# noveens/reviews4rec

Measured on AMD Instinct MI355X. Metric: train ratings/sec, higher is better.
Workload: dtype f32

## Files before the change

### include/r4r.h

```cpp
#ifndef R4R_H
#define R4R_H

#include <stddef.h>
#include <stdint.h>

#ifdef __cplusplus
extern "C" {
#endif

#define R4R_OK 0
#define R4R_ERR_ARG (-1)
#define R4R_ERR_LAUNCH (-2)
#define R4R_ERR_WORKSPACE (-3)

int r4r_version(void);
const char *r4r_last_error(void);

size_t r4r_textcnn_ws_bytes(int64_t N, int T, int E, int F, int64_t V);
int r4r_textcnn_fwd(const float *table, int64_t V, const int64_t *idx,
                    const float *conv_w, const float *conv_b,
                    float *pooled, int32_t *argmax,
                    void *ws, size_t ws_bytes,
                    int64_t N, int T, int E, int F, void *stream);

// ... 27 lines not shown
int r4r_add(const float *a, const float *b, float *out, int64_t n, void *stream);

int r4r_fm_fwd(const float *x, const float *V, const float *lin_w, const float *lin_b,
               float *out, int64_t N, int n, int k, void *stream);
int r4r_fm_bwd(const float *x, const float *V, const float *lin_w, const float *g_out,
               float *g_x, float *g_V, float *g_lin_w, float *g_lin_b,
               int64_t N, int n, int k, void *stream);

int r4r_embed_gather(const float *table, const int64_t *idx, float *out,
                     int64_t R, int D, int64_t n, void *stream);
int r4r_embed_scatter_add(const float *g_out, const int64_t *idx, float *g_table,
                          int64_t R, int D, int64_t n, void *stream);
int r4r_embed_scatter_add_ordered(const float *g_out, const int64_t *idx, float *g_table,
                                  int64_t R, int D, int64_t n, void *stream);

int r4r_rowdot_fwd(const float *a, const float *c, float *out, int64_t N, int D, void *stream);
int r4r_rowdot_bwd(const float *a, const float *c, const float *g_out, float *g_a, float *g_c,
                   int64_t N, int D, void *stream);
int r4r_bias_head_fwd(const float *r, const float *user_bias, const float *item_bias,
                      const float *global_bias, const int64_t *uid, const int64_t *iid,
                      float *out, int64_t N, void *stream);
int r4r_bias_head_bwd(const float *g_out, const int64_t *uid, const int64_t *iid,
                      float *g_user_bias, float *g_item_bias, float *g_global,
                      int64_t RU, int64_t RI, int64_t N, void *stream);

size_t r4r_narre_attn_ws_bytes(int64_t N, int R, int L);
int r4r_narre_attn_fwd(const float *x, const float *other, const float *W0, const float *b0,
                       const float *w3, const float *b3, const float *mult,
                       float *out, float *h_save, float *a_save,
                       int64_t N, int R, int L, void *stream);
int r4r_narre_attn_bwd(const float *x, const float *other, const float *W0, const float *w3,
                       const float *mult, const float *h_save, const float *a_save,
                       const float *g_out,
                       float *g_x, float *g_other, float *g_W0, float *g_b0, float *g_w3, float *g_b3,
                       void *ws, size_t ws_bytes,
                       int64_t N, int R, int L, void *stream);

int r4r_mse_fwd_bwd(const float *out, const float *y, float *se, float *g_out,
                    int64_t N, float denom, void *stream);

int r4r_sqdist_mean_fwd(const float *a, const float *b, float *out, int64_t N, int L, void *stream);
int r4r_sqdist_mean_bwd(const float *a, const float *b, const float *g_out, float *g_a, float *g_b,
                        int64_t N, int L, void *stream);

int r4r_adam_chunk_elems(void);
int r4r_adam_multi(int ntensor, const uint64_t *p, const uint64_t *g, const uint64_t *m, const uint64_t *v,
                   const int64_t *numel, float lr, double beta1, double beta2, float eps,
                   float weight_decay, int64_t step, const int64_t *step_dev, void *stream);
int r4r_adam_gathered(float *p, const float *gathered, int world, float *g_sum, float *m, float *v,
                      int64_t numel, float lr, double beta1, double beta2, float eps,
                      float weight_decay, int64_t step, void *stream);
int r4r_adam_gathered_guarded(float *p, const float *gathered, int world, float *g_sum, float *m, float *v,
                              int64_t numel, float lr, double beta1, double beta2, float eps,
                              float weight_decay, int64_t step, const uint32_t *abort_word, void *stream);

int r4r_peer_segment_create(int64_t bytes, void **ptr, uint8_t *handle);
int r4r_peer_segment_open(const uint8_t *handle, void **ptr);
int r4r_peer_segment_close(void *ptr);
int r4r_peer_segment_destroy(void *ptr);
int r4r_peer_push(const float *src, int64_t numel, const uint64_t *peer_dst, const uint64_t *peer_flags,
                  uint32_t *arrive, int rank, int world, uint32_t epoch, const uint32_t *wait_flags,
                  uint32_t *timed_out, double timeout_s, void *stream);
int r4r_peer_wait(const uint32_t *flags, int world, uint32_t epoch, uint32_t *timed_out, double timeout_s, void *stream);


#define R4R_CONV_AUTO 0
#define R4R_CONV_DIRECT 1
#define R4R_CONV_PROJECT 2
int r4r_deepconn_nparam(void);
int r4r_deepconn_layout(int E, int L, int64_t *offsets, int64_t *sizes, int64_t *total);
size_t r4r_deepconn_ws_bytes(int64_t B, int T, int E, int L, int64_t V);
size_t r4r_deepconn_ws_mult_offset(int64_t B, int T, int E, int L, int64_t V);
size_t r4r_deepconn_ws_count_offset(int64_t B, int T, int E, int L, int64_t V, int tower, int buffer);
int r4r_deepconn_step(const float *table, int64_t V, const int64_t *user_idx, const int64_t *item_idx,
                      const float *y, float *flat_p, float *flat_g,
                      float *pred, float *se, float *sse_accum,
                      void *ws, size_t ws_bytes,
                      int64_t B, int T, int E, int L,
                      float dropout_p, int training, uint64_t seed, uint64_t offset,
                      float inv_denom, int conv_algo, int token_buffer, int tokens_ready,
                      const int64_t *next_user_idx, const int64_t *next_item_idx,
                      float *flat_m, float *flat_v, float lr, double beta1, double beta2, float eps,
                      float weight_decay, int64_t adam_step, void *stream);
int r4r_deepconn_tokens(const int64_t *user_idx, const int64_t *item_idx, void *ws, size_t ws_bytes,
                        int64_t B, int T, int E, int L, int64_t V, int conv_algo, int token_buffer,
                        int discard, void *stream);

#define R4R_TIMING_TEXTCNN_FWD 0
#define R4R_TIMING_TEXTCNN_WGRAD 1
#define R4R_TIMING_ADAM 2
#define R4R_TIMING_PROJ_GEMM 3
#define R4R_TIMING_PROJ_GATHER 4
#define R4R_TIMING_SLOTS 8
int r4r_timing_enable(int slot_mask);
int r4r_timing_read(int slot, double *total_ms, int64_t *count, int reset);

size_t r4r_mf_ws_bytes(int64_t B, int D, int64_t n_users, int64_t n_items);
size_t r4r_mf_ws_persist_bytes(int64_t B, int D, int64_t n_users, int64_t n_items);
size_t r4r_mf_ws_mult_offset(int64_t B, int D, int64_t n_users, int64_t n_items);
size_t r4r_mf_ws_grad_offset(int64_t B, int D, int64_t n_users, int64_t n_items, int which);
int r4r_mf_step(const int64_t *uid, const int64_t *iid, const float *y,
                const uint64_t *p, const uint64_t *m, const uint64_t *v,
                int64_t n_users, int64_t n_items, int D,
                float *pred, float *se, float *sse_accum, void *ws, size_t ws_bytes, int64_t B,
                float dropout_p, int training, uint64_t seed, uint64_t offset, float inv_denom,
                int sweep_period, int64_t sweep_base, int sweep_all,
                float lr, double beta1, double beta2, float eps, float weight_decay, int64_t adam_step,
                void *stream);

int r4r_mf_rows_flush(const uint64_t *p, const uint64_t *m, const uint64_t *v,
                      int64_t n_users, int64_t n_items, int D, void *ws, size_t ws_bytes, int64_t B,
                      int sweep_period, int64_t sweep_base,
                      float lr, double beta1, double beta2, float eps, float weight_decay, int64_t adam_step,
                      void *stream);
size_t r4r_mf_ws_flag_offset(int64_t B, int D, int64_t n_users, int64_t n_items);

int r4r_sse_accumulate(const float *se, int64_t n, float *accum, void *stream);

size_t r4r_mf_dp_block_bytes(int64_t B_pad, int D);
int r4r_mf_grad(const int64_t *uid, const int64_t *iid, const float *y, const uint64_t *p,
                const uint64_t *m, const uint64_t *v,
                int64_t n_users, int64_t n_items, int D, float *pred, float *se, void *block, float *mult,
                int64_t B, int64_t B_pad, float dropout_p, int training, uint64_t seed, uint64_t offset,
                float inv_denom, void *ws, int sweep_period, int64_t sweep_base,
                float lr, double beta1, double beta2, float eps, float weight_decay, int64_t adam_step,
                void *stream);
int r4r_mf_apply(const void *blocks, int world, int64_t B_pad, const uint64_t *p, const uint64_t *m,
                 const uint64_t *v, int64_t n_users, int64_t n_items, int D, void *ws, size_t ws_bytes,
                 int sweep_period, int64_t sweep_base, int sweep_all,
                 const float *se, int64_t se_n, float *sse_accum,
                 float lr, double beta1, double beta2, float eps, float weight_decay, int64_t adam_step,
                 void *stream);
int r4r_mf_grad_push(const int64_t *uid, const int64_t *iid, const float *y, const uint64_t *p,
                     const uint64_t *m, const uint64_t *v,
                     int64_t n_users, int64_t n_items, int D, float *pred, float *se, float *mult,
                     int64_t B, int64_t B_pad, float dropout_p, int training, uint64_t seed, uint64_t offset,
                     float inv_denom, void *ws, int sweep_period, int64_t sweep_base,
                     float lr, double beta1, double beta2, float eps, float weight_decay, int64_t adam_step,
                     const uint64_t *peer_dst, const uint64_t *peer_flags, uint32_t *arrive, int rank, int world,
                     uint32_t epoch, void *stream);
int r4r_mf_apply_peer(const void *blocks, int world, int64_t B_pad, const uint64_t *p, const uint64_t *m,
                      const uint64_t *v, int64_t n_users, int64_t n_items, int D, void *ws, size_t ws_bytes,
                      int sweep_period, int64_t sweep_base, int sweep_all,
                      const float *se, int64_t se_n, float *sse_accum,
                      float lr, double beta1, double beta2, float eps, float weight_decay, int64_t adam_step,
                      const uint32_t *wait_flags, uint32_t epoch, uint32_t *timed_out, double timeout_s,
                      void *stream);

size_t r4r_dp_block_bytes(int nfields, const int *widths, int64_t B_pad);
int r4r_dp_pack(int nfields, const uint64_t *src, const int *widths, const int *pad_ones, int64_t n,
                int64_t B_pad, void *block, void *stream);
int r4r_dp_unpack(int nfields, const uint64_t *dst, const int *widths, const void *blocks, int world,
                  int64_t B_pad, void *stream);

int r4r_narre_nparam(void);
int r4r_narre_layout(int E, int L, int64_t *offsets, int64_t *sizes, int64_t *total);
size_t r4r_narre_ws_bytes(int64_t B, int R, int T, int E, int L, int64_t V, int64_t n_users, int64_t n_items);
size_t r4r_narre_ws_offset(int64_t B, int R, int T, int E, int L, int64_t V, int64_t n_users, int64_t n_items,
                           int which);
int r4r_narre_step(const float *table, int64_t V,
                   const int64_t *user_reviews, const int64_t *item_reviews,
                   const int64_t *reviewed_items, const int64_t *users_who_reviewed,
                   const int64_t *uid, const int64_t *iid, const float *y,
                   float *flat_p, float *flat_g, float *flat_m, float *flat_v,
                   const uint64_t *rows_p, const uint64_t *rows_m, const uint64_t *rows_v,
                   int64_t n_users, int64_t n_items,
// ... 295 lines not shown
```

### reviews4rec_amd/csrc/engine.hip

```cpp
#include <stdlib.h>

#include "trace_device.h"
#include "textcnn.h"
#include "wgrad_device.h"
#include "tokens_device.h"
#include "adam_device.h"

namespace r4r {

constexpr int F_CONV = 100;
constexpr int FM_K = 8;
constexpr int MAX_L = 128;

enum { P_UCW = 0, P_UCB, P_UFW, P_UFB, P_ICW, P_ICB, P_IFW, P_IFB, P_FMV, P_FMLW, P_FMLB, P_GB, P_COUNT };

struct Layout {
    int64_t off[P_COUNT], size[P_COUNT], total;
};

static Layout make_layout(int E, int L) {
    Layout lay;
    const int64_t sz[P_COUNT] = {(int64_t)F_CONV * 3 * E, F_CONV, (int64_t)L * F_CONV, L,
                                 (int64_t)F_CONV * 3 * E, F_CONV, (int64_t)L * F_CONV, L,
                                 (int64_t)2 * L * FM_K, 2 * L, 1, 1};
    int64_t o = 0;
    for (int i = 0; i < P_COUNT; ++i) {
        lay.off[i] = o;
        lay.size[i] = sz[i];
        o += (sz[i] + 31) & ~(int64_t)31;
    }
    lay.total = o;
    return lay;
}

struct HeadArgs {
    const float *pmax[2]; const int *parg[2];
    const float *fc_w[2]; const float *fc_b[2];
    const float *V, *lin_w, *lin_b, *gbias;
    const float *y;
    float *pooled[2]; int *argmax[2];
    float *g_pooled[2];
    float *mult;
    float *x, *s, *g, *gz;
    float *pred, *se;
    int64_t B;
    int L, tiles, training, want_grad;
    float p_drop, inv_denom;
    uint64_t seed, offset;
};


constexpr int HEAD_MAX_TILES = 8;

#define SEL2(arr, s) ((s) ? (arr)[1] : (arr)[0])
HEAD_TRACE_DEFINE(r4r_debug_dc_head_trace)
template <int ML>
__global__ __launch_bounds__(256) void deepconn_head_wg_kernel(HeadArgs a) {
    HEAD_STAMP(0)
    constexpr int N2 = 2 * ML, PARTS = 256 / N2;
    __shared__ float sw[2][ML][F_CONV + 1];
    __shared__ float sfb[N2], slw[N2], sz[N2];
    __shared__ float sV[N2][FM_K];
    __shared__ float sp[2][F_CONV + 4];
    __shared__ float red[N2][PARTS + 1];
    const int tid = threadIdx.x, lane = tid & 63, w = tid >> 6;
    const int64_t b = blockIdx.x;
    const int L = a.L, n = 2 * L;
    const float lin_b0 = a.lin_b[0], gbias0 = a.gbias[0], yb = a.y ? a.y[b] : 0.f;

    constexpr int FQ = F_CONV / 4;
    typedef float hq4 __attribute__((ext_vector_type(4)));
    constexpr int WREGS = (2 * ML * FQ + 255) / 256;
    hq4 wreg[WREGS];
    const int wtot = 2 * L * FQ;
#pragma unroll
    for (int k = 0; k < WREGS; ++k) {
        const int i = min(tid + 256 * k, wtot - 1);
        const int t = i >= L * FQ;
        wreg[k] = *reinterpret_cast<const hq4 *>(SEL2(a.fc_w, t) + 4 * (i - t * L * FQ));
    }
    const int tn = min(tid, n - 1);
    const float fbreg = SEL2(a.fc_b, tn >= L)[tn - (tn >= L ? L : 0)];
    const float lwreg = a.lin_w[tn];
    constexpr int VREGS = (N2 * FM_K + 255) / 256;
    float vreg[VREGS];
#pragma unroll
    for (int k = 0; k < VREGS; ++k) vreg[k] = a.V[min(tid + 256 * k, n * FM_K - 1)];

    {
        const int t = w >> 1, f = lane + 64 * (w & 1), fc = min(f, F_CONV - 1);
        float best = -INFINITY;
        int bp = -1;
        if (a.tiles <= HEAD_MAX_TILES) {
            float v[HEAD_MAX_TILES];
            int pp[HEAD_MAX_TILES];
#pragma unroll
            for (int k = 0; k < HEAD_MAX_TILES; ++k) {
                const size_t o = ((size_t)b * a.tiles + min(k, a.tiles - 1)) * NP + fc;
                v[k] = SEL2(a.pmax, t)[o];
                pp[k] = SEL2(a.parg, t)[o];
            }
#pragma unroll
            for (int k = 0; k < HEAD_MAX_TILES; ++k)
                if (v[k] > best) { best = v[k]; bp = pp[k]; }
        } else {
            for (int k0 = 0; k0 < a.tiles; k0 += HEAD_MAX_TILES) {
                float v[HEAD_MAX_TILES];
                int pp[HEAD_MAX_TILES];
#pragma unroll
                for (int k = 0; k < HEAD_MAX_TILES; ++k) {
                    const bool in = k0 + k < a.tiles;
                    const size_t o = ((size_t)b * a.tiles + (in ? k0 + k : 0)) * NP + fc;
                    v[k] = in ? SEL2(a.pmax, t)[o] : -INFINITY;
                    pp[k] = SEL2(a.parg, t)[o];
                }
#pragma unroll
                for (int k = 0; k < HEAD_MAX_TILES; ++k)
                    if (v[k] > best) { best = v[k]; bp = pp[k]; }
            }
        }
        if (!(best > 0.f)) { best = 0.f; bp = -1; }
        if (f < F_CONV) {
            sp[t][f] = best;
            SEL2(a.pooled, t)[b * F_CONV + f] = best;
            SEL2(a.argmax, t)[b * F_CONV + f] = bp;
        }
    }
    HEAD_STAMP(1)
#pragma unroll
    for (int k = 0; k < WREGS; ++k) {
        const int i = tid + 256 * k;
        if (i < wtot) {
            const int t = i >= L * FQ, r = i - t * L * FQ, l = r / FQ, f0 = 4 * (r - l * FQ);
#pragma unroll
            for (int c = 0; c < 4; ++c) sw[t][l][f0 + c] = wreg[k][c];
        }
    }
    if (tid < n) { sfb[tid] = fbreg; slw[tid] = lwreg; }
#pragma unroll
    for (int k = 0; k < VREGS; ++k) {
// ... 31 lines not shown
            if (a.training && a.p_drop > 0.f && i < n) {
                const uint32_t r = philox_first_word(a.offset + (uint64_t)(b * n + i), a.seed);
                const float uu = (float)(r >> 8) * (1.0f / 16777216.0f);
                mult[u] = (uu >= a.p_drop) ? 1.f / (1.f - a.p_drop) : 0.f;
            }
            xi[u] *= mult[u];
        }
        float inter = 0.f;
        float sk_keep[FM_K];
#pragma unroll
        for (int k = 0; k < FM_K; ++k) {
            float pv = 0.f, pv2 = 0.f, vv[NI];
#pragma unroll
            for (int u = 0; u < NI; ++u) {
                const int i = lane + 64 * u;
                vv[u] = (i < n) ? sV[i][k] : 0.f;
                pv += xi[u] * vv[u];
                pv2 += xi[u] * xi[u] * vv[u] * vv[u];
            }
            const float sk = wave_sum(pv);
            const float s2 = wave_sum(pv2);
            inter += sk * sk - s2;
#pragma unroll
            for (int u = 0; u < NI; ++u) gacc[u] += sk * vv[u] - xi[u] * vv[u] * vv[u];
            sk_keep[k] = sk;
        }
        float pl = 0.f;
#pragma unroll
        for (int u = 0; u < NI; ++u) pl += xi[u] * lw[u];
        const float lin = wave_sum(pl);
        const float pred = (0.5f * inter + lin + lin_b0) + gbias0;
        if (lane == 0) a.pred[b] = pred;
        if (has_y) {
            const float d = pred - yb;
            if (lane == 0) a.se[b] = d * d;
            if (want) {
                const float g = 2.f * d * a.inv_denom;
#pragma unroll
                for (int u = 0; u < NI; ++u) {
                    const int i = lane + 64 * u;
                    const float gx = g * (gacc[u] + lw[u]);
                    const float gz = gx * mult[u];
                    if (i < n) {
                        sz[i] = gz;
                        a.x[b * n + i] = xi[u];
                        a.gz[b * n + i] = gz;
                        a.mult[b * n + i] = mult[u];
                    }
                }
                if (lane < FM_K) {
                    float sv = 0.f;
#pragma unroll
                    for (int k = 0; k < FM_K; ++k) if (lane == k) sv = sk_keep[k];
                    a.s[b * FM_K + lane] = sv;
                }
                if (lane == 0) a.g[b] = g;
            }
        }
    }
    if (!want) return;
    __syncthreads();
    HEAD_STAMP(3)
    if (tid < 2 * F_CONV) {
        const int t = tid >= F_CONV, f = tid - t * F_CONV;
        float acc = 0.f;
        for (int l = 0; l < L; ++l) acc = fmaf(sz[t * L + l], sw[t][l][f], acc);
        SEL2(a.g_pooled, t)[b * F_CONV + f] = acc;
    }
    HEAD_STAMP(4)
}

struct HeadGradArgs {
    const float *pooled[2];
    const float *x, *s, *g, *gz;
    const float *V;
    const float *se;
    float *g_fc_w[2], *g_fc_b[2], *g_V, *g_lin_w, *g_lin_b, *g_gb;
    float *sse_accum;
    int64_t B;
    int L;
};

constexpr int HG_ROWS = 16, HG_COLS = 16;
__device__ __forceinline__ void head_grad_block(const HeadGradArgs &a, int blk) {
    __shared__ float red[HG_ROWS][HG_COLS];
    const int ox = threadIdx.x & (HG_COLS - 1), rg = threadIdx.x / HG_COLS;
    const int L = a.L, n = 2 * L;
    const int n_fcw = L * F_CONV;
    const int seg[9] = {n_fcw, L, n_fcw, L, n * FM_K, n, 1, 1, 1};
    int o = blk * HG_COLS + ox;
    int which = -1, local = 0, acc_o = o;
#pragma unroll
    for (int k = 0; k < 9; ++k) {
        if (which < 0) {
            if (acc_o < seg[k]) { which = k; local = acc_o; }
            else acc_o -= seg[k];
        }
    }
    float s = 0.f;
    if (which >= 0) {
        const bool is_w = which == 0 || which == 2, is_b = which == 1 || which == 3, is_v = which == 4, is_lw = which == 5;
        const int t = which >> 1;
        const int wl = local / F_CONV, wf = local - wl * F_CONV;
        const int vi = local / FM_K, vk = local - vi * FM_K;
        const float *pa = (is_w || is_b) ? a.gz : (which == 8 ? a.se : a.g);
        const int64_t sa = (is_w || is_b) ? n : 1;
        const int64_t oa = is_w ? t * L + wl : (is_b ? t * L + local : 0);
        const bool useb = is_w || is_v, usec = is_v || is_lw;
        const float *pb = is_w ? a.pooled[t & 1] : (is_v ? a.s : a.g);
        const int64_t sb = is_w ? F_CONV : (is_v ? FM_K : 1), ob = is_w ? wf : (is_v ? vk : 0);
        const float *pc = usec ? a.x : a.g;
        const int64_t sc = usec ? n : 1, oc = is_v ? vi : (is_lw ? local : 0);
        const float cv = is_v ? a.V[local] : 0.f;
        constexpr int HB = 8;
        for (int64_t b0 = rg; b0 < a.B; b0 += (int64_t)HG_ROWS * HB) {
            float va[HB], vb[HB], vc[HB];
#pragma unroll
            for (int k = 0; k < HB; ++k) {
                const int64_t b = min(b0 + (int64_t)k * HG_ROWS, a.B - 1);
                va[k] = pa[b * sa + oa];
                vb[k] = pb[b * sb + ob];
                vc[k] = pc[b * sc + oc];
            }
#pragma unroll
            for (int k = 0; k < HB; ++k) {
                const float B_ = useb ? vb[k] : 1.f, C_ = usec ? vc[k] : 1.f;
                const float term = va[k] * (B_ * C_ - C_ * C_ * cv);
                if (b0 + (int64_t)k * HG_ROWS < a.B) s += term;
            }
        }
    }
    red[rg][ox] = s;
    __syncthreads();
    if (rg == 0 && which >= 0) {
        float t = 0.f;
#pragma unroll
        for (int r = 0; r < HG_ROWS; ++r) t += red[r][ox];
        switch (which) {
            case 0: a.g_fc_w[0][local] = t; break;
            case 1: a.g_fc_b[0][local] = t; break;
            case 2: a.g_fc_w[1][local] = t; break;
            case 3: a.g_fc_b[1][local] = t; break;
            case 4: a.g_V[local] = t; break;
            case 5: a.g_lin_w[local] = t; break;
            case 6: a.g_lin_b[0] = t; break;
            case 7: a.g_gb[0] = t; break;
            default: if (a.sse_accum) a.sse_accum[0] += t; break;
        }
    }
}

BWD_TRACE_DEFINE(r4r_debug_dc_bwd_trace)
struct DcBackwardArgs {
    WgradArgs w;
    HeadGradArgs h;
    int hg_blocks;
    TokenArgs nx;
};
__global__ __launch_bounds__(WG_THREADS, 8) void deepconn_backward_kernel(DcBackwardArgs) {
    const DcBackwardArgs &A = kernel_args<DcBackwardArgs>();
    const WgradArgs &w = A.w;
    const HeadGradArgs &h = A.h;
    const TokenArgs &nx = A.nx;
    const int hg_blocks = A.hg_blocks;
    BWD_STAMP(0, wall_clock64())
    BWD_STAMP(2, (unsigned long long)blockIdx.z + 1)
    if (blockIdx.z == 1 || blockIdx.z == 2) {
        wgrad_block(w, blockIdx.x, blockIdx.y, blockIdx.z - 1);
    } else if (blockIdx.z == 0) {
        for (int blk = blockIdx.y * gridDim.x + blockIdx.x; blk < hg_blocks; blk += gridDim.x * gridDim.y) {
            head_grad_block(h, blk);
            __syncthreads();
        }
    } else {
        token_mark_block(nx, blockIdx.y * gridDim.x + blockIdx.x, gridDim.x * gridDim.y, WG_THREADS);
    }
#ifdef R4R_TRACE
    __syncthreads();
#endif
    BWD_STAMP(1, wall_clock64())
}

constexpr int RED_THREADS = 256;
struct FusedAdam {
    float *p, *m, *v;
    const float *g;
    int64_t lo[2], hi[2];
    AdamScalars s;
    int on;
};
__global__ __launch_bounds__(RED_THREADS) void deepconn_reduce_kernel(WgradArgs w, int red_blocks, int comp_blocks,
                                                                      TokenArgs nx, FusedAdam opt) {
    const int bx = blockIdx.x;
    if (bx < red_blocks) {
        const WgradTower &tw = w.t[blockIdx.y];
        const int nw = w.F * 3 * w.E;
        const int i = bx * RED_THREADS + threadIdx.x;
        const float *gp0 = i < nw ? tw.d_w + i : (i < nw + w.F ? tw.d_b + (i - nw) : nullptr);
        const int64_t o = gp0 ? gp0 - opt.g : 0;
        float P = 0.f, M = 0.f, V = 0.f;
        if (opt.on && gp0) { P = opt.p[o]; M = opt.m[o]; V = opt.v[o]; }
        float *dst;
        const float g = wgrad_reduce_elem(w, blockIdx.y, i, dst);
        if (opt.on && dst) {
            adam_elem(P, g, M, V, opt.s);
            opt.p[o] = P; opt.m[o] = M; opt.v[o] = V;
        }
    } else if (bx < red_blocks + comp_blocks) {
        token_compact_auto<RED_THREADS / 64>(nx.t[blockIdx.y], nx.V, bx - red_blocks);
    } else {
        const int64_t o = opt.lo[blockIdx.y] + (int64_t)(bx - red_blocks - comp_blocks) * RED_THREADS + threadIdx.x;
        if (o < opt.hi[blockIdx.y]) {
            float P = opt.p[o], M = opt.m[o], V = opt.v[o];
            adam_elem(P, opt.g[o], M, V, opt.s);
            opt.p[o] = P; opt.m[o] = M; opt.v[o] = V;
        }
    }
}

__global__ void sse_only_kernel(const float *__restrict__ se, float *__restrict__ accum, int64_t B) {
    __shared__ float red[256];
    float s = 0.f;
    for (int64_t i = threadIdx.x; i < B; i += 256) s += se[i];
    red[threadIdx.x] = s;
    __syncthreads();
    for (int off = 128; off > 0; off >>= 1) {
        if ((int)threadIdx.x < off) red[threadIdx.x] += red[threadIdx.x + off];
        __syncthreads();
    }
    if (threadIdx.x == 0) accum[0] += red[0];
}

struct StepWs {
    float *wp[2], *pmax[2]; int *parg[2];
    int *flags[2][2], *slot[2][2], *list[2][2], *count[2][2]; float *ptab[2];
    float *pooled[2]; int *argmax[2]; float *g_pooled[2];
    float *mult, *x, *s, *g, *gz;
    float *part_w[2], *part_b[2];
    size_t bytes;
};

static StepWs carve(void *ws, int64_t B, int T, int E, int L, int64_t V) {
    StepWs w;
    char *p = static_cast<char *>(ws);
    auto take = [&](size_t nbytes) { char *r = p; p += align256(nbytes); return r; };
    const size_t tiles128 = (size_t)(T + 2 + 127) / 128;
    const int ns = textcnn_wgrad_splits(B);
    for (int t = 0; t < 2; ++t) {
        w.wp[t] = reinterpret_cast<float *>(take(textcnn_wp_floats(E) * 4));
        w.pmax[t] = reinterpret_cast<float *>(take((size_t)B * tiles128 * NP * 4));
        w.parg[t] = reinterpret_cast<int *>(take((size_t)B * tiles128 * NP * 4));
        w.pooled[t] = reinterpret_cast<float *>(take((size_t)B * F_CONV * 4));
        w.argmax[t] = reinterpret_cast<int *>(take((size_t)B * F_CONV * 4));
        w.g_pooled[t] = reinterpret_cast<float *>(take((size_t)B * F_CONV * 4));
        w.part_w[t] = reinterpret_cast<float *>(take((size_t)ns * F_CONV * 3 * E * 4));
        w.part_b[t] = reinterpret_cast<float *>(take((size_t)ns * F_CONV * 4));
        for (int bf = 0; bf < 2; ++bf) {
            w.flags[bf][t] = reinterpret_cast<int *>(take((size_t)(V + 4) * 4));
            w.slot[bf][t] = reinterpret_cast<int *>(take((size_t)(V + 4) * 4));
            w.list[bf][t] = reinterpret_cast<int *>(take((size_t)proj_row_capacity(B, T, V) * 4));
            w.count[bf][t] = reinterpret_cast<int *>(take(256));
        }
        w.ptab[t] = reinterpret_cast<float *>(take(proj_ptab_floats(B, T, V) * 4));
    }
    w.mult = reinterpret_cast<float *>(take((size_t)B * 2 * L * 4));
    w.x = reinterpret_cast<float *>(take((size_t)B * 2 * L * 4));
    w.gz = reinterpret_cast<float *>(take((size_t)B * 2 * L * 4));
    w.s = reinterpret_cast<float *>(take((size_t)B * FM_K * 4));
    w.g = reinterpret_cast<float *>(take((size_t)B * 4));
    w.bytes = (size_t)(p - static_cast<char *>(ws));
    return w;
}

}

using namespace r4r;

extern "C" int r4r_deepconn_nparam(void) { return P_COUNT; }

extern "C" int r4r_deepconn_layout(int E, int L, int64_t *offsets, int64_t *sizes, int64_t *total) {
    R4R_REQUIRE(E > 0 && L > 0 && L <= MAX_L && offsets && sizes && total, "deepconn_layout: bad arguments");
    const Layout lay = make_layout(E, L);
    for (int i = 0; i < P_COUNT; ++i) { offsets[i] = lay.off[i]; sizes[i] = lay.size[i]; }
    *total = lay.total;
    return R4R_OK;
}

extern "C" size_t r4r_deepconn_ws_bytes(int64_t B, int T, int E, int L, int64_t V) {
    if (B < 0 || T <= 0 || E <= 0 || L <= 0 || V <= 0) return 0;
    return carve(nullptr, B, T, E, L, V).bytes;
}

extern "C" size_t r4r_deepconn_ws_mult_offset(int64_t B, int T, int E, int L, int64_t V) {
    char base[1];
    const StepWs w = carve(base, B, T, E, L, V);
    return (size_t)(reinterpret_cast<char *>(w.mult) - base);
}

extern "C" size_t r4r_deepconn_ws_count_offset(int64_t B, int T, int E, int L, int64_t V, int tower, int buffer) {
    char base[1];
    const StepWs w = carve(base, B, T, E, L, V);
    return (size_t)(reinterpret_cast<char *>(w.count[buffer & 1][tower & 1]) - base);
}

extern "C" int r4r_deepconn_tokens(const int64_t *user_idx, const int64_t *item_idx, void *ws, size_t ws_bytes,
                                   int64_t B, int T, int E, int L, int64_t V, int conv_algo, int token_buffer,
                                   int discard, void *stream) {
    R4R_REQUIRE(user_idx && item_idx && ws, "deepconn_tokens: null pointer");
    R4R_REQUIRE(token_buffer == 0 || token_buffer == 1, "deepconn_tokens: token_buffer must be 0 or 1");
    if (ws_bytes < r4r_deepconn_ws_bytes(B, T, E, L, V)) {
        set_error("deepconn_tokens: workspace %zu < %zu bytes", ws_bytes, r4r_deepconn_ws_bytes(B, T, E, L, V));
        return R4R_ERR_WORKSPACE;
    }
    if (B == 0 || textcnn_pick_algo(conv_algo, B, T, E, F_CONV) != R4R_CONV_PROJECT) return R4R_OK;
    const StepWs w = carve(ws, B, T, E, L, V);
    if (discard) {
        for (int t = 0; t < 2; ++t) (void)hipMemsetAsync(w.count[token_buffer][t], 0, sizeof(int), as_stream(stream));
        return check_launch("deepconn_tokens(discard)");
    }
    ProjTower pt[2];
    const int64_t *idx[2] = {user_idx, item_idx};
    for (int t = 0; t < 2; ++t) {
        pt[t] = ProjTower{};
        pt[t].idx = idx[t];
        pt[t].flags = w.flags[token_buffer][t]; pt[t].slot = w.slot[token_buffer][t];
        pt[t].list = w.list[token_buffer][t]; pt[t].count = w.count[token_buffer][t];
    }
    return textcnn_proj_tokens_launch(V, pt, 2, B, T, false, as_stream(stream));
}

extern "C" int r4r_deepconn_step(const float *table, int64_t V, const int64_t *user_idx, const int64_t *item_idx,
                                 const float *y, float *flat_p, float *flat_g,
                                 float *pred, float *se, float *sse_accum,
                                 void *ws, size_t ws_bytes,
                                 int64_t B, int T, int E, int L,
                                 float dropout_p, int training, uint64_t seed, uint64_t offset,
                                 float inv_denom, int conv_algo, int token_buffer, int tokens_ready,
                                 const int64_t *next_user_idx, const int64_t *next_item_idx,
                                 float *flat_m, float *flat_v, float lr, double beta1, double beta2, float eps,
                                 float weight_decay, int64_t adam_step,
                                 void *stream) {
    R4R_REQUIRE(table && user_idx && item_idx && flat_p && pred && ws, "deepconn_step: null pointer");
    R4R_REQUIRE(!flat_m == !flat_v, "deepconn_step: flat_m and flat_v go together");
    R4R_REQUIRE(!flat_m || (flat_g && adam_step >= 1), "deepconn_step: the fused optimiser needs gradients and "
                                                       "adam_step >= 1");
    R4R_REQUIRE(!next_user_idx == !next_item_idx, "deepconn_step: next_user_idx and next_item_idx go together");
    R4R_REQUIRE(!next_user_idx || flat_g, "deepconn_step: the next batch's tokens ride on the backward launches "
                                          "(training steps only)");
    R4R_REQUIRE(V > 0 && B >= 0 && T > 0, "deepconn_step: bad sizes");
    R4R_REQUIRE(E > 0 && E % 4 == 0, "deepconn_step: word_embed_size %d must be a positive multiple of 4", E);
    R4R_REQUIRE(L > 0 && L <= MAX_L, "deepconn_step: latent_size %d outside 1..%d", L, MAX_L);
    R4R_REQUIRE(!flat_g || (y && se), "deepconn_step: gradients need ratings y and the se buffer");
    R4R_REQUIRE(!y || se, "deepconn_step: se buffer required when y is given");
    R4R_REQUIRE(dropout_p >= 0.f && dropout_p < 1.f, "deepconn_step: dropout %f outside [0,1)", (double)dropout_p);
    R4R_REQUIRE(B * (int64_t)((T + 2 + 127) / 128) < (1ll << 31), "deepconn_step: grid too large");
    R4R_REQUIRE(token_buffer == 0 || token_buffer == 1, "deepconn_step: token_buffer must be 0 or 1");
    if (ws_bytes < r4r_deepconn_ws_bytes(B, T, E, L, V)) {
        set_error("deepconn_step: workspace %zu < %zu bytes", ws_bytes, r4r_deepconn_ws_bytes(B, T, E, L, V));
        return R4R_ERR_WORKSPACE;
    }
    if (B == 0) return R4R_OK;
    hipStream_t st = as_stream(stream);
    const Layout lay = make_layout(E, L);
    const StepWs w = carve(ws, B, T, E, L, V);
    const float *P[P_COUNT];
    float *G[P_COUNT];
    for (int i = 0; i < P_COUNT; ++i) {
        P[i] = flat_p + lay.off[i];
        G[i] = flat_g ? flat_g + lay.off[i] : nullptr;
    }

    const int64_t *idx[2] = {user_idx, item_idx};
    const int algo = textcnn_pick_algo(conv_algo, B, T, E, F_CONV);
    int tiles;
    if (algo == R4R_CONV_PROJECT) {
        ProjTower pt[2];
        for (int t = 0; t < 2; ++t) {
            pt[t].idx = idx[t];
            pt[t].conv_w = P[t ? P_ICW : P_UCW];
            pt[t].conv_b = P[t ? P_ICB : P_UCB];
            pt[t].flags = w.flags[token_buffer][t]; pt[t].slot = w.slot[token_buffer][t];
            pt[t].list = w.list[token_buffer][t]; pt[t].count = w.count[token_buffer][t];
            pt[t].ptab = w.ptab[t]; pt[t].pmax = w.pmax[t]; pt[t].parg = w.parg[t]; pt[t].wimg = w.wp[t];
        }
        if (!tokens_ready)
            if (int rc = textcnn_proj_tokens_launch(V, pt, 2, B, T, false, st)) return rc;
        if (int rc = textcnn_proj_compute_launch(table, V, pt, 2, B, T, E, F_CONV, st)) return rc;
        tiles = proj_tiles(T);
    } else {
        FwdTower ft[2];
        for (int t = 0; t < 2; ++t) {
            ft[t].idx = idx[t];
            ft[t].conv_w = P[t ? P_ICW : P_UCW];
            ft[t].conv_b = P[t ? P_ICB : P_UCB];
            ft[t].wp = w.wp[t]; ft[t].pmax = w.pmax[t]; ft[t].parg = w.parg[t];
        }
        if (int rc = textcnn_fwd_launch(table, ft, 2, B, T, E, F_CONV, st)) return rc;
        tiles = textcnn_tiles(T);
    }

    HeadArgs h;
    for (int t = 0; t < 2; ++t) {
        h.pmax[t] = w.pmax[t]; h.parg[t] = w.parg[t];
        h.fc_w[t] = P[t ? P_IFW : P_UFW]; h.fc_b[t] = P[t ? P_IFB : P_UFB];
        h.pooled[t] = w.pooled[t]; h.argmax[t] = w.argmax[t]; h.g_pooled[t] = w.g_pooled[t];
    }
    h.V = P[P_FMV]; h.lin_w = P[P_FMLW]; h.lin_b = P[P_FMLB]; h.gbias = P[P_GB];
    h.y = y; h.mult = w.mult; h.x = w.x; h.s = w.s; h.g = w.g; h.gz = w.gz;
    h.pred = pred; h.se = se;
    h.B = B; h.L = L; h.tiles = tiles; h.training = training; h.want_grad = flat_g != nullptr;
    h.p_drop = dropout_p; h.inv_denom = inv_denom; h.seed = seed; h.offset = offset;
    if (L <= 16) deepconn_head_wg_kernel<16><<<(unsigned)B, 256, 0, st>>>(h);
    else if (L <= 32) deepconn_head_wg_kernel<32><<<(unsigned)B, 256, 0, st>>>(h);
    else if (L <= 64) deepconn_head_wg_kernel<64><<<(unsigned)B, 256, 0, st>>>(h);
    else deepconn_head_wg_kernel<128><<<(unsigned)B, 256, 0, st>>>(h);

    if (!flat_g) {
        if (y && sse_accum) sse_only_kernel<<<1, 256, 0, st>>>(se, sse_accum, B);
        return check_launch("deepconn_step(forward)");
    }

    HeadGradArgs hg;
    for (int t = 0; t < 2; ++t) {
        hg.pooled[t] = w.pooled[t];
        hg.g_fc_w[t] = G[t ? P_IFW : P_UFW]; hg.g_fc_b[t] = G[t ? P_IFB : P_UFB];
    }
    hg.x = w.x; hg.s = w.s; hg.g = w.g; hg.gz = w.gz; hg.V = P[P_FMV]; hg.se = se;
    hg.g_V = G[P_FMV]; hg.g_lin_w = G[P_FMLW]; hg.g_lin_b = G[P_FMLB]; hg.g_gb = G[P_GB];
    hg.sse_accum = sse_accum; hg.B = B; hg.L = L;
    const int nout = 2 * (L * F_CONV + L) + 2 * L * FM_K + 2 * L + 3;
    const int hg_blocks = (nout + HG_COLS - 1) / HG_COLS;

    WgradTower wt[2];
    WgradArgs wa;
    for (int t = 0; t < 2; ++t) {
        wt[t].idx = idx[t]; wt[t].g_pooled = w.g_pooled[t]; wt[t].argmax = w.argmax[t];
        wt[t].part_w = w.part_w[t]; wt[t].part_b = w.part_b[t];
        wt[t].d_w = G[t ? P_ICW : P_UCW]; wt[t].d_b = G[t ? P_ICB : P_UCB];
    }
    for (int k = 0; k < MAX_TOWERS; ++k) wa.t[k] = wt[k < 2 ? k : 0];
    wa.table = table; wa.N = B; wa.T = T; wa.E = E; wa.F = F_CONV;
    wa.table_bytes = (int64_t)V * E * 4;
    wa.nsplit = textcnn_wgrad_splits(B);
    wa.per_split = (int)cdiv(B, wa.nsplit);
    const bool prefetch = next_user_idx && algo == R4R_CONV_PROJECT;
    TokenArgs nx{};
    if (prefetch) {
        ProjTower nt[2];
        const int64_t *nidx[2] = {next_user_idx, next_item_idx};
        const int ob = token_buffer ^ 1;
        for (int t = 0; t < 2; ++t) {
            nt[t] = ProjTower{};
            nt[t].idx = nidx[t];
            nt[t].flags = w.flags[ob][t]; nt[t].slot = w.slot[ob][t];
            nt[t].list = w.list[ob][t]; nt[t].count = w.count[ob][t];
        }
        nx = make_token_args(V, nt, 2, B, T);
    }
    {
        ScopedTiming tm(R4R_TIMING_TEXTCNN_WGRAD, st);
        deepconn_backward_kernel<<<dim3(F_CONV, wa.nsplit, prefetch ? 4 : 3), WG_THREADS, 0, st>>>(DcBackwardArgs{wa, hg, hg_blocks, nx});
    }
    const int red_blocks = (F_CONV * 3 * E + F_CONV + RED_THREADS - 1) / RED_THREADS;
    const int comp_blocks = prefetch ? (int)cdiv((V + 3) / 4, RED_THREADS * compact_groups(V)) : 0;
    FusedAdam opt{};
    int opt_blocks = 0;
    if (flat_m) {
        opt.on = 1;
        opt.p = flat_p; opt.m = flat_m; opt.v = flat_v; opt.g = flat_g;
        opt.lo[0] = lay.off[P_UFW]; opt.hi[0] = lay.off[P_ICW];
        opt.lo[1] = lay.off[P_IFW]; opt.hi[1] = lay.total;
        opt.s = adam_make_scalars(lr, beta1, beta2, eps, weight_decay, adam_step, nullptr);
        const int64_t longest = opt.hi[0] - opt.lo[0] > opt.hi[1] - opt.lo[1] ? opt.hi[0] - opt.lo[0] : opt.hi[1] - opt.lo[1];
        opt_blocks = (int)cdiv(longest, RED_THREADS);
    }
    deepconn_reduce_kernel<<<dim3(red_blocks + comp_blocks + opt_blocks, 2), RED_THREADS, 0, st>>>(
        wa, red_blocks, comp_blocks, nx, opt);
    return check_launch("deepconn_step");
}

extern "C" int r4r_sse_accumulate(const float *se, int64_t n, float *accum, void *stream) {
    R4R_REQUIRE(accum && (se || n == 0) && n >= 0, "sse_accumulate: bad arguments");
    if (n == 0) return R4R_OK;
    sse_only_kernel<<<1, 256, 0, as_stream(stream)>>>(se, accum, n);
    return check_launch("sse_accumulate");
}
```

### reviews4rec_amd/csrc/wgrad_device.h

```cpp
#pragma once
#include "textcnn.h"

namespace r4r {

typedef float wg_f32x4 __attribute__((ext_vector_type(4)));

constexpr int WG_THREADS = 256;

struct WgradArgs {
    WgradTower t[MAX_TOWERS];
    const float *table;
    int64_t N;
    int T, E, F, per_split, nsplit;
    int64_t table_bytes = 0;
};

constexpr int WG_CHUNK = 16;
constexpr int WG_FLIGHT = 8;

template <bool FIRST>
__device__ __forceinline__ void wgrad_block_pass(const WgradArgs &a, int f, int s, int tower, int v0,
                                                 long (&s_off)[WG_CHUNK][3], float (&s_g)[WG_CHUNK]) {
    const WgradTower &tw = a.t[tower];
    const float *__restrict__ table = a.table;
    const int64_t *__restrict__ idx = tw.idx;
    const float *__restrict__ gp = tw.g_pooled;
    const int *__restrict__ argmax = tw.argmax;
    const int T = a.T, E = a.E, F = a.F;
    const int64_t n0 = (int64_t)s * a.per_split;
    const int64_t n1 = min(a.N, n0 + (int64_t)a.per_split);
    const int nvec = 3 * E / 4;
    const int tid = threadIdx.x;
    wg_f32x4 acc[2] = {(wg_f32x4){0.f, 0.f, 0.f, 0.f}, (wg_f32x4){0.f, 0.f, 0.f, 0.f}};
    int vj[2], ve[2];
#pragma unroll
    for (int k = 0; k < 2; ++k) {
        const int v = v0 + tid + k * WG_THREADS;
        vj[k] = (v * 4) / E;
        ve[k] = v * 4 - vj[k] * E;
    }
    float sb = 0.f;
    const bool buf_ok = a.table_bytes > 0 && a.table_bytes < (1ll << 32);
    const __amdgpu_buffer_rsrc_t rsrc = __builtin_amdgcn_make_buffer_rsrc(const_cast<float *>(table), 0, buf_ok ? (int)(unsigned)a.table_bytes : 0, 0x00020000);
    for (int64_t c0 = n0; c0 < n1; c0 += WG_CHUNK) {
        const int nd = (int)min((int64_t)WG_CHUNK, n1 - c0);
        __syncthreads();
        if (tid < nd * 3) {
            const int d = tid / 3, j = tid - d * 3;
            const int64_t n = c0 + d;
            const int p = argmax[n * F + f];
            const float gv = gp[n * F + f];
            const int t = p - 2 + j;
            long off = -1;
            if (p >= 0 && t >= 0 && t < T) off = (long)idx[n * T + t] * E;
            s_off[d][j] = off;
            if (j == 0) s_g[d] = (p >= 0) ? gv : 0.f;
        }
        __syncthreads();
        if (buf_ok) {
#pragma unroll
            for (int k = 0; k < 2; ++k) {
                if (v0 + tid + k * WG_THREADS < nvec) {
#pragma unroll
                    for (int d0 = 0; d0 < WG_CHUNK; d0 += WG_FLIGHT) {
                        wg_f32x4 row[WG_FLIGHT];
                        bool on[WG_FLIGHT];
#pragma unroll
                        for (int u = 0; u < WG_FLIGHT; ++u) {
                            const int d = d0 + u;
                            const long off = d < nd ? s_off[d][vj[k]] : -1;
                            on[u] = off >= 0;
                            const unsigned bo = on[u] ? (unsigned)((off + ve[k]) * 4) : 0xfffffff0u;
                            row[u] = __builtin_bit_cast(wg_f32x4, __builtin_amdgcn_raw_buffer_load_b128(rsrc, (int)bo, 0, 0));
                        }
#pragma unroll
                        for (int u = 0; u < WG_FLIGHT; ++u) {
                            const wg_f32x4 sum = acc[k] + s_g[d0 + u < nd ? d0 + u : 0] * row[u];
                            acc[k] = on[u] ? sum : acc[k];
                        }
                    }
                }
            }
        } else {
#pragma unroll
// ... 54 lines not shown
        if (live) {
            int pv[NRES];
            float gv[NRES];
#pragma unroll
            for (int k = 0; k < NRES; ++k) {
                const int i = lane + 64 * k, d = i / 3;
                const int64_t n = c0 + (d < nd ? d : 0);
                pv[k] = argmax[n * F + f];
                gv[k] = gp[n * F + f];
                if (d >= nd) pv[k] = -1;
            }
            long off[NRES], tokv[NRES];
            bool onv[NRES];
#pragma unroll
            for (int k = 0; k < NRES; ++k) {
                const int i = lane + 64 * k, d = i / 3, j = i - d * 3;
                const int64_t n = c0 + (d < nd ? d : 0);
                const int t = pv[k] - 2 + j;
                onv[k] = pv[k] >= 0 && t >= 0 && t < T;
                tokv[k] = idx[n * T + (onv[k] ? t : 0)];
            }
#pragma unroll
            for (int k = 0; k < NRES; ++k) asm volatile("" : "+v"(tokv[k]));
#pragma unroll
            for (int k = 0; k < NRES; ++k) off[k] = onv[k] ? tokv[k] * E : -1;
#pragma unroll
            for (int k = 0; k < NRES; ++k) {
                const int i = lane + 64 * k, d = i / 3, j = i - d * 3;
                if (d < WG_SUPER) {
                    p_off[wave][d][j] = off[k];
                    if (j == 0) p_g[wave][d] = pv[k] >= 0 ? gv[k] : 0.f;
                }
            }
        }
        __syncthreads();
        if (live && lane < nvec) {
            for (int r0 = 0; r0 < nd; r0 += WG_CHUNK) {
                wg_f32x4 v[WG_CHUNK];
#pragma unroll
                for (int d = 0; d < WG_CHUNK; ++d) {
                    const long off = p_off[wave][r0 + d][vj];
                    v[d] = *reinterpret_cast<const wg_f32x4 *>(table + (off < 0 ? 0 : off) + ve);
                }
#pragma unroll
                for (int d = 0; d < WG_CHUNK; ++d) {
                    const wg_f32x4 sum = acc + p_g[wave][r0 + d] * v[d];
                    acc = p_off[wave][r0 + d][vj] >= 0 ? sum : acc;
                }
            }
        }
        if (live && lane == 0)
            for (int d = 0; d < nd; ++d) sb += p_g[wave][d];
    }
    if (live && lane < nvec) *reinterpret_cast<wg_f32x4 *>(tw.part_w + ((size_t)s * F + f) * 3 * E + lane * 4) = acc;
    if (live && lane == 0) tw.part_b[(size_t)s * F + f] = sb;
}

constexpr int WG_MAX_SPLITS = 16;

__device__ __forceinline__ float wgrad_reduce_elem(const WgradArgs &a, int tower, int i, float *&dst) {
    const WgradTower &tw = a.t[tower];
    const int nw = a.F * 3 * a.E;
    const float *src;
    size_t stride;
    if (i < nw) { src = tw.part_w + i; stride = (size_t)nw; dst = tw.d_w + i; }
    else if (i < nw + a.F) { src = tw.part_b + (i - nw); stride = (size_t)a.F; dst = tw.d_b + (i - nw); }
    else { dst = nullptr; return 0.f; }
    float v[WG_MAX_SPLITS];
#pragma unroll
    for (int k = 0; k < WG_MAX_SPLITS; ++k) v[k] = src[(size_t)(k < a.nsplit ? k : 0) * stride];
    float s = 0.f;
#pragma unroll
    for (int k = 0; k < WG_MAX_SPLITS; ++k)
        if (k < a.nsplit) s += v[k];
    *dst = s;
    return s;
}

__device__ __forceinline__ void wgrad_reduce_block(const WgradArgs &a, int tower, int blk) {
    float *dst;
    (void)wgrad_reduce_elem(a, tower, blk * (int)blockDim.x + (int)threadIdx.x, dst);
}

}
```

Before: 1.389 million.

## Fuse DeepCoNN backward tail: in-block split reduction, Adam, and token marking

Replaces the backward kernel plus separate reduce/Adam kernel with one fused kernel. Each block reduces all batch splits for its filter column slice in shared memory, applying Adam to conv and head gradients in place. Token marking for the next batch moves into extra blocks of the head kernel. This removes a kernel launch and the global round-trip of split partials, at the cost of larger blocks (up to 1024 threads) and a different parallel decomposition for the wgrad gather.

```diff
diff --git a/include/r4r.h b/include/r4r.h
--- a/include/r4r.h
+++ b/include/r4r.h
@@ -133,6 +133,8 @@
                       const int64_t *next_user_idx, const int64_t *next_item_idx,
                       float *flat_m, float *flat_v, float lr, double beta1, double beta2, float eps,
                       float weight_decay, int64_t adam_step, void *stream);
+int r4r_deepconn_tail_mode(int mode);
+int r4r_deepconn_last_launches(void);
 int r4r_deepconn_tokens(const int64_t *user_idx, const int64_t *item_idx, void *ws, size_t ws_bytes,
                         int64_t B, int T, int E, int L, int64_t V, int conv_algo, int token_buffer,
                         int discard, void *stream);
diff --git a/reviews4rec_amd/csrc/engine.hip b/reviews4rec_amd/csrc/engine.hip
--- a/reviews4rec_amd/csrc/engine.hip
+++ b/reviews4rec_amd/csrc/engine.hip
@@ -47,6 +47,8 @@
     int L, tiles, training, want_grad;
     float p_drop, inv_denom;
     uint64_t seed, offset;
+    int mark_blocks;
+    TokenArgs nx;
 };
 
 
@@ -56,6 +58,11 @@
 HEAD_TRACE_DEFINE(r4r_debug_dc_head_trace)
 template <int ML>
 __global__ __launch_bounds__(256) void deepconn_head_wg_kernel(HeadArgs a) {
+    if ((int64_t)blockIdx.x >= a.B) {
+        const HeadArgs &A = kernel_args<HeadArgs>();
+        token_mark_block(A.nx, (int)(blockIdx.x - a.B), A.mark_blocks, 256);
+        return;
+    }
     HEAD_STAMP(0)
     constexpr int N2 = 2 * ML, PARTS = 256 / N2;
     __shared__ float sw[2][ML][F_CONV + 1];
@@ -253,7 +260,7 @@
 };
 
 constexpr int HG_ROWS = 16, HG_COLS = 16;
-__device__ __forceinline__ void head_grad_block(const HeadGradArgs &a, int blk) {
+__device__ __forceinline__ void head_grad_block(const HeadGradArgs &a, int blk, const FusedAdam *opt = nullptr) {
     __shared__ float red[HG_ROWS][HG_COLS];
     const int ox = threadIdx.x & (HG_COLS - 1), rg = threadIdx.x / HG_COLS;
     const int L = a.L, n = 2 * L;
@@ -269,6 +276,18 @@
         }
     }
     float s = 0.f;
+    const bool upd = opt && opt->on && rg == 0 && which >= 0 && which < 8;
+    int64_t po = 0;
+    float P = 0.f, M = 0.f, V = 0.f;
+    if (upd) {
+        const int64_t so[8] = {a.g_fc_w[0] - opt->g, a.g_fc_b[0] - opt->g, a.g_fc_w[1] - opt->g, a.g_fc_b[1] - opt->g,
+                               a.g_V - opt->g, a.g_lin_w - opt->g, a.g_lin_b - opt->g, a.g_gb - opt->g};
+        int64_t base = so[7];
+#pragma unroll
+        for (int k = 6; k >= 0; --k) base = which == k ? so[k] : base;
+        po = base + local;
+        P = opt->p[po]; M = opt->m[po]; V = opt->v[po];
+    }
     if (which >= 0) {
         const bool is_w = which == 0 || which == 2, is_b = which == 1 || which == 3, is_v = which == 4, is_lw = which == 5;
         const int t = which >> 1;
@@ -317,6 +336,10 @@
             case 6: a.g_lin_b[0] = t; break;
             case 7: a.g_gb[0] = t; break;
             default: if (a.sse_accum) a.sse_accum[0] += t; break;
+        }
+        if (upd) {
+            adam_elem(P, t, M, V, opt->s);
+            opt->p[po] = P; opt->m[po] = M; opt->v[po] = V;
         }
     }
 }
@@ -352,14 +375,37 @@
     BWD_STAMP(1, wall_clock64())
 }
 
+struct DcTailArgs {
+    WgradArgs w;
+    HeadGradArgs h;
+    int hg_blocks, nparts, comp_blocks;
+    TokenArgs nx;
+    FusedAdam opt;
+};
+__global__ __launch_bounds__(64 * WG_MAX_SPLITS, 8) void deepconn_backward_fused_kernel(DcTailArgs) {
+    const DcTailArgs &A = kernel_args<DcTailArgs>();
+    if (blockIdx.z == 1 || blockIdx.z == 2) {
+        wgrad_fused_block(A.w, blockIdx.x, blockIdx.y, A.nparts, blockIdx.z - 1, A.opt);
+        return;
+    }
+    if (threadIdx.x >= 256) return;
+    const int nblk = gridDim.x * gridDim.y;
+    if (blockIdx.z == 0) {
+        const int hg_blocks = A.hg_blocks;
+        for (int blk = blockIdx.y * gridDim.x + blockIdx.x; blk < hg_blocks; blk += nblk) {
+            head_grad_block(A.h, blk, &A.opt);
+            __syncthreads();
+        }
+    } else {
+        const int comp_blocks = A.comp_blocks, ntower = A.nx.ntower;
+        for (int blk = blockIdx.y * gridDim.x + blockIdx.x; blk < comp_blocks * ntower; blk += nblk) {
+            token_compact_auto<4>(A.nx.t[blk / comp_blocks], A.nx.V, blk % comp_blocks);
+            __syncthreads();
+        }
+    }
+}
+
 constexpr int RED_THREADS = 256;
-struct FusedAdam {
-    float *p, *m, *v;
-    const float *g;
-    int64_t lo[2], hi[2];
-    AdamScalars s;
-    int on;
-};
 __global__ __launch_bounds__(RED_THREADS) void deepconn_reduce_kernel(WgradArgs w, int red_blocks, int comp_blocks,
                                                                       TokenArgs nx, FusedAdam opt) {
     const int bx = blockIdx.x;
@@ -499,6 +545,21 @@
     }
     return textcnn_proj_tokens_launch(V, pt, 2, B, T, false, as_stream(stream));
 }
+
+static int g_tail_mode = -1;
+static int g_last_launches = 0;
+static int tail_mode() {
+    if (g_tail_mode < 0) {
+        const char *e = getenv("R4R_DC_TAIL");
+        g_tail_mode = (e && e[0] == 's') ? 1 : 0;
+    }
+    return g_tail_mode;
+}
+extern "C" int r4r_deepconn_tail_mode(int mode) {
+    if (mode == 0 || mode == 1) g_tail_mode = mode;
+    return tail_mode();
+}
+extern "C" int r4r_deepconn_last_launches(void) { return g_last_launches; }
 
 extern "C" int r4r_deepconn_step(const float *table, int64_t V, const int64_t *user_idx, const int64_t *item_idx,
                                  const float *y, float *flat_p, float *flat_g,
@@ -544,6 +605,7 @@
     const int64_t *idx[2] = {user_idx, item_idx};
     const int algo = textcnn_pick_algo(conv_algo, B, T, E, F_CONV);
     int tiles;
+    int launches = 2;
     if (algo == R4R_CONV_PROJECT) {
         ProjTower pt[2];
         for (int t = 0; t < 2; ++t) {
@@ -554,8 +616,10 @@
             pt[t].list = w.list[token_buffer][t]; pt[t].count = w.count[token_buffer][t];
             pt[t].ptab = w.ptab[t]; pt[t].pmax = w.pmax[t]; pt[t].parg = w.parg[t]; pt[t].wimg = w.wp[t];
         }
-        if (!tokens_ready)
+        if (!tokens_ready) {
             if (int rc = textcnn_proj_tokens_launch(V, pt, 2, B, T, false, st)) return rc;
+            launches += 2;
+        }
         if (int rc = textcnn_proj_compute_launch(table, V, pt, 2, B, T, E, F_CONV, st)) return rc;
         tiles = proj_tiles(T);
     } else {
@@ -581,40 +645,11 @@
     h.pred = pred; h.se = se;
     h.B = B; h.L = L; h.tiles = tiles; h.training = training; h.want_grad = flat_g != nullptr;
     h.p_drop = dropout_p; h.inv_denom = inv_denom; h.seed = seed; h.offset = offset;
-    if (L <= 16) deepconn_head_wg_kernel<16><<<(unsigned)B, 256, 0, st>>>(h);
-    else if (L <= 32) deepconn_head_wg_kernel<32><<<(unsigned)B, 256, 0, st>>>(h);
-    else if (L <= 64) deepconn_head_wg_kernel<64><<<(unsigned)B, 256, 0, st>>>(h);
-    else deepconn_head_wg_kernel<128><<<(unsigned)B, 256, 0, st>>>(h);
-
-    if (!flat_g) {
-        if (y && sse_accum) sse_only_kernel<<<1, 256, 0, st>>>(se, sse_accum, B);
-        return check_launch("deepconn_step(forward)");
-    }
-
-    HeadGradArgs hg;
-    for (int t = 0; t < 2; ++t) {
-        hg.pooled[t] = w.pooled[t];
-        hg.g_fc_w[t] = G[t ? P_IFW : P_UFW]; hg.g_fc_b[t] = G[t ? P_IFB : P_UFB];
-    }
-    hg.x = w.x; hg.s = w.s; hg.g = w.g; hg.gz = w.gz; hg.V = P[P_FMV]; hg.se = se;
-    hg.g_V = G[P_FMV]; hg.g_lin_w = G[P_FMLW]; hg.g_lin_b = G[P_FMLB]; hg.g_gb = G[P_GB];
-    hg.sse_accum = sse_accum; hg.B = B; hg.L = L;
-    const int nout = 2 * (L * F_CONV + L) + 2 * L * FM_K + 2 * L + 3;
-    const int hg_blocks = (nout + HG_COLS - 1) / HG_COLS;
-
-    WgradTower wt[2];
-    WgradArgs wa;
-    for (int t = 0; t < 2; ++t) {
-        wt[t].idx = idx[t]; wt[t].g_pooled = w.g_pooled[t]; wt[t].argmax = w.argmax[t];
-        wt[t].part_w = w.part_w[t]; wt[t].part_b = w.part_b[t];
-        wt[t].d_w = G[t ? P_ICW : P_UCW]; wt[t].d_b = G[t ? P_ICB : P_UCB];
-    }
-    for (int k = 0; k < MAX_TOWERS; ++k) wa.t[k] = wt[k < 2 ? k : 0];
-    wa.table = table; wa.N = B; wa.T = T; wa.E = E; wa.F = F_CONV;
-    wa.table_bytes = (int64_t)V * E * 4;
-    wa.nsplit = textcnn_wgrad_splits(B);
-    wa.per_split = (int)cdiv(B, wa.nsplit);
-    const bool prefetch = next_user_idx && algo == R4R_CONV_PROJECT;
+    const int nsplit = textcnn_wgrad_splits(B);
+    const int64_t table_bytes = (int64_t)V * E * 4;
+    const bool fused = flat_g && tail_mode() == 0 && 3 * E / 4 > 64 && 3 * E / 4 <= 2 * WG_THREADS &&
+                       nsplit <= WG_MAX_SPLITS && table_bytes < (1ll << 32);
+    const bool prefetch = flat_g && next_user_idx && algo == R4R_CONV_PROJECT;
     TokenArgs nx{};
     if (prefetch) {
         ProjTower nt[2];
@@ -628,25 +663,82 @@
         }
         nx = make_token_args(V, nt, 2, B, T);
     }
+    h.mark_blocks = 0;
+    h.nx = nx;
+    if (fused && prefetch) {
+        int mb = (int)cdiv(B * T * 2, 256 * 8);
+        h.mark_blocks = mb > 1024 ? 1024 : (mb < 1 ? 1 : mb);
+    }
+    const unsigned head_grid = (unsigned)(B + h.mark_blocks);
+    if (L <= 16) deepconn_head_wg_kernel<16><<<head_grid, 256, 0, st>>>(h);
+    else if (L <= 32) deepconn_head_wg_kernel<32><<<head_grid, 256, 0, st>>>(h);
+    else if (L <= 64) deepconn_head_wg_kernel<64><<<head_grid, 256, 0, st>>>(h);
+    else deepconn_head_wg_kernel<128><<<head_grid, 256, 0, st>>>(h);
+    ++launches;
+
+    if (!flat_g) {
+        if (y && sse_accum) { sse_only_kernel<<<1, 256, 0, st>>>(se, sse_accum, B); ++launches; }
+        g_last_launches = launches;
+        return check_launch("deepconn_step(forward)");
+    }
+
+    HeadGradArgs hg;
+    for (int t = 0; t < 2; ++t) {
+        hg.pooled[t] = w.pooled[t];
+        hg.g_fc_w[t] = G[t ? P_IFW : P_UFW]; hg.g_fc_b[t] = G[t ? P_IFB : P_UFB];
+    }
+    hg.x = w.x; hg.s = w.s; hg.g = w.g; hg.gz = w.gz; hg.V = P[P_FMV]; hg.se = se;
+    hg.g_V = G[P_FMV]; hg.g_lin_w = G[P_FMLW]; hg.g_lin_b = G[P_FMLB]; hg.g_gb = G[P_GB];
+    hg.sse_accum = sse_accum; hg.B = B; hg.L = L;
+    const int nout = 2 * (L * F_CONV + L) + 2 * L * FM_K + 2 * L + 3;
+    const int hg_blocks = (nout + HG_COLS - 1) / HG_COLS;
+
+    WgradTower wt[2];
+    WgradArgs wa;
+    for (int t = 0; t < 2; ++t) {
+        wt[t].idx = idx[t]; wt[t].g_pooled = w.g_pooled[t]; wt[t].argmax = w.argmax[t];
+        wt[t].part_w = w.part_w[t]; wt[t].part_b = w.part_b[t];
+        wt[t].d_w = G[t ? P_ICW : P_UCW]; wt[t].d_b = G[t ? P_ICB : P_UCB];
+    }
+    for (int k = 0; k < MAX_TOWERS; ++k) wa.t[k] = wt[k < 2 ? k : 0];
+    wa.table = table; wa.N = B; wa.T = T; wa.E = E; wa.F = F_CONV;
+    wa.table_bytes = table_bytes;
+    wa.nsplit = nsplit;
+    wa.per_split = (int)cdiv(B, wa.nsplit);
+    const int comp_blocks = prefetch ? (int)cdiv((V + 3) / 4, RED_THREADS * compact_groups(V)) : 0;
+    FusedAdam opt{};
+    if (flat_m) {
+        opt.on = 1;
+        opt.p = flat_p; opt.m = flat_m; opt.v = flat_v;
+        opt.lo[0] = lay.off[P_UFW]; opt.hi[0] = lay.off[P_ICW];
+        opt.lo[1] = lay.off[P_IFW]; opt.hi[1] = lay.total;
+        opt.s = adam_make_scalars(lr, beta1, beta2, eps, weight_decay, adam_step, nullptr);
+    }
+    opt.g = flat_g;
+    if (fused) {
+        const int nparts = wgrad_fused_parts(E);
+        const int threads = wgrad_fused_threads(E, nsplit);
+        {
+            ScopedTiming tm(R4R_TIMING_TEXTCNN_WGRAD, st);
+            deepconn_backward_fused_kernel<<<dim3(F_CONV, nparts, prefetch ? 4 : 3), threads, 0, st>>>(
+                DcTailArgs{wa, hg, hg_blocks, nparts, comp_blocks, nx, opt});
+        }
+        g_last_launches = launches + 1;
+        return check_launch("deepconn_step");
+    }
     {
         ScopedTiming tm(R4R_TIMING_TEXTCNN_WGRAD, st);
         deepconn_backward_kernel<<<dim3(F_CONV, wa.nsplit, prefetch ? 4 : 3), WG_THREADS, 0, st>>>(DcBackwardArgs{wa, hg, hg_blocks, nx});
     }
     const int red_blocks = (F_CONV * 3 * E + F_CONV + RED_THREADS - 1) / RED_THREADS;
-    const int comp_blocks = prefetch ? (int)cdiv((V + 3) / 4, RED_THREADS * compact_groups(V)) : 0;
-    FusedAdam opt{};
     int opt_blocks = 0;
     if (flat_m) {
-        opt.on = 1;
-        opt.p = flat_p; opt.m = flat_m; opt.v = flat_v; opt.g = flat_g;
-        opt.lo[0] = lay.off[P_UFW]; opt.hi[0] = lay.off[P_ICW];
-        opt.lo[1] = lay.off[P_IFW]; opt.hi[1] = lay.total;
-        opt.s = adam_make_scalars(lr, beta1, beta2, eps, weight_decay, adam_step, nullptr);
         const int64_t longest = opt.hi[0] - opt.lo[0] > opt.hi[1] - opt.lo[1] ? opt.hi[0] - opt.lo[0] : opt.hi[1] - opt.lo[1];
         opt_blocks = (int)cdiv(longest, RED_THREADS);
     }
     deepconn_reduce_kernel<<<dim3(red_blocks + comp_blocks + opt_blocks, 2), RED_THREADS, 0, st>>>(
         wa, red_blocks, comp_blocks, nx, opt);
+    g_last_launches = launches + 2;
     return check_launch("deepconn_step");
 }
 
diff --git a/reviews4rec_amd/csrc/wgrad_device.h b/reviews4rec_amd/csrc/wgrad_device.h
--- a/reviews4rec_amd/csrc/wgrad_device.h
+++ b/reviews4rec_amd/csrc/wgrad_device.h
@@ -1,5 +1,6 @@
 #pragma once
 #include "textcnn.h"
+#include "adam_device.h"
 
 namespace r4r {
 
@@ -220,4 +221,107 @@
     (void)wgrad_reduce_elem(a, tower, blk * (int)blockDim.x + (int)threadIdx.x, dst);
 }
 
-}
+struct FusedAdam {
+    float *p, *m, *v;
+    const float *g;
+    int64_t lo[2], hi[2];
+    AdamScalars s;
+    int on;
+};
+
+constexpr int WGF_COLS = 64;
+constexpr int WGF_ROW = WGF_COLS * 4 + 4;
+static inline int wgrad_fused_parts(int E) { return (3 * E / 4 + WGF_COLS - 1) / WGF_COLS; }
+static inline int wgrad_fused_threads(int E, int nsplit) {
+    const int nvec = 3 * E / 4, nparts = wgrad_fused_parts(E), pw = (nvec + nparts - 1) / nparts;
+    const int owners = (4 * pw + 1 + 63) / 64;
+    return 64 * (nsplit > owners ? nsplit : owners);
+}
+
+__device__ __forceinline__ void wgrad_fused_block(const WgradArgs &a, int f, int part, int nparts, int tower,
+                                                  const FusedAdam &opt) {
+    __shared__ long s_off[WG_MAX_SPLITS][WG_CHUNK][3];
+    __shared__ float s_g[WG_MAX_SPLITS][WG_CHUNK];
+    __shared__ float s_part[WG_MAX_SPLITS][WGF_ROW];
+    const WgradTower &tw = a.t[tower];
+    const int64_t *__restrict__ idx = tw.idx;
+    const float *__restrict__ gp = tw.g_pooled;
+    const int *__restrict__ argmax = tw.argmax;
+    const int T = a.T, E = a.E, F = a.F, nsplit = a.nsplit;
+    const int tid = threadIdx.x, lane = tid & 63, s = tid >> 6;
+    const int nvec = 3 * E / 4;
+    const int pw = (nvec + nparts - 1) / nparts;
+    const int c0 = part * pw, ncol = max(0, min(pw, nvec - c0));
+    const bool adam = opt.on != 0;
+
+    const bool own_w = tid < 4 * ncol, own = own_w || (part == 0 && tid == 4 * ncol);
+    float *const gdst = own_w ? tw.d_w + ((size_t)f * 3 * E + 4 * c0 + tid) : tw.d_b + f;
+    const int po = (int)(gdst - opt.g);
+    float P = 0.f, M = 0.f, V = 0.f;
+    if (adam && own) { P = opt.p[po]; M = opt.m[po]; V = opt.v[po]; }
+
+    const int N = (int)a.N;
+    const int n0 = min(N, s * a.per_split);
+    const int n1 = s < nsplit ? min(N, n0 + a.per_split) : n0;
+    const bool colv = lane < ncol;
+    const int v = c0 + (colv ? lane : 0);
+    const int vj = (v * 4) / E, ve = v * 4 - vj * E;
+    wg_f32x4 acc = (wg_f32x4){0.f, 0.f, 0.f, 0.f};
+    float sb = 0.f;
+    const __amdgpu_buffer_rsrc_t rsrc = __builtin_amdgcn_make_buffer_rsrc(const_cast<float *>(a.table), 0, (int)(unsigned)a.table_bytes, 0x00020000);
+    for (int d00 = n0; d00 < n1; d00 += WG_CHUNK) {
+        const int nd = min(WG_CHUNK, n1 - d00);
+        wave_lds_fence();
+        if (lane < nd * 3) {
+            const int d = lane / 3, j = lane - d * 3;
+            const int64_t n = d00 + d;
+            const int p = argmax[n * F + f];
+            const float gv = gp[n * F + f];
+            const int t = p - 2 + j;
+            long off = -1;
+            if (p >= 0 && t >= 0 && t < T) off = (long)idx[n * T + t] * E;
+            s_off[s][d][j] = off;
+            if (j == 0) s_g[s][d] = (p >= 0) ? gv : 0.f;
+        }
+        wave_lds_fence();
+        if (colv) {
+#pragma unroll 1
+            for (int d0 = 0; d0 < WG_CHUNK; d0 += WG_FLIGHT) {
+                wg_f32x4 row[WG_FLIGHT];
+                bool on[WG_FLIGHT];
+#pragma unroll
+                for (int u = 0; u < WG_FLIGHT; ++u) {
+                    const int d = d0 + u;
+                    const long off = d < nd ? s_off[s][d][vj] : -1;
+                    on[u] = off >= 0;
+                    const unsigned bo = on[u] ? (unsigned)((off + ve) * 4) : 0xfffffff0u;
+                    row[u] = __builtin_bit_cast(wg_f32x4, __builtin_amdgcn_raw_buffer_load_b128(rsrc, (int)bo, 0, 0));
+                }
+#pragma unroll
+                for (int u = 0; u < WG_FLIGHT; ++u) {
+                    const wg_f32x4 sum = acc + s_g[s][d0 + u < nd ? d0 + u : 0] * row[u];
+                    acc = on[u] ? sum : acc;
+                }
+            }
+        }
+        if (part == 0 && lane == 0)
+            for (int d = 0; d < nd; ++d) sb += s_g[s][d];
+    }
+    if (colv) *reinterpret_cast<wg_f32x4 *>(&s_part[s][lane * 4]) = acc;
+    if (lane == 0) s_part[s][4 * ncol] = sb;
+    __syncthreads();
+
+    if (own) {
+        float g = 0.f;
+#pragma unroll
+        for (int k = 0; k < WG_MAX_SPLITS; ++k)
+            if (k < nsplit) g += s_part[k][tid];
+        *gdst = g;
+        if (adam) {
+            adam_elem(P, g, M, V, opt.s);
+            opt.p[po] = P; opt.m[po] = M; opt.v[po] = V;
+        }
+    }
+}
+
+}
```

Result: slower. 1.212 million (-12.7%).
